# tusen-ai/simpledet

Measured on AMD Instinct MI355X. Metric: images/sec at 800x1333 FPN 512-RoI RoIAlign fwd+bwd, higher is better.
Workload: dtype f32; 1 GPU; fused FPN RoIAlign_v2 fwd+bwd, P2-P5 256ch 800x1333, N=2 img/GPU, 512 RoIs/img, 7x7x4 samples (BASELINE configs[1]); images_per_gpu=2, rois_per_image=512, argmax_state=packed u8 (decoded in backward)

## Files before the change

simpledet_amd/csrc/common.h:

```cpp
#pragma once
#include <hip/hip_runtime.h>
#include <stdint.h>
#include <stdio.h>
#include <stdarg.h>

#define SD_OK 0
#define SD_ERR_INVALID_ARG (-1)
#define SD_ERR_UNSUPPORTED (-2)
#define SD_ERR_HIP (-3)
#define SD_ERR_WORKSPACE (-4)

namespace sd {

char* err_buf();
int fail(int code, const char* fmt, ...);
void note_dispatch(const char* fmt, ...);

#define SD_REQUIRE(cond, ...)                                    \
  do {                                                           \
    if (!(cond)) return ::sd::fail(SD_ERR_INVALID_ARG, __VA_ARGS__); \
  } while (0)

#define SD_HIP_CHECK(expr)                                                              \
  do {                                                                                  \
    hipError_t e_ = (expr);                                                             \
    if (e_ != hipSuccess)                                                               \
      return ::sd::fail(SD_ERR_HIP, "%s failed: %s (%s:%d)", #expr, hipGetErrorString(e_), \
                        __FILE__, __LINE__);                                            \
  } while (0)

#define SD_LAUNCH_CHECK() SD_HIP_CHECK(hipGetLastError())

int tuning(const char* key, int dflt);
#ifdef SD_PROFILING
#define SD_PROF_TUNING(key, dflt) ::sd::tuning(key, dflt)
#define SD_ABLATE(args, bits) ((args).ablate & (bits))
#else
#define SD_PROF_TUNING(key, dflt) (dflt)
#define SD_ABLATE(args, bits) 0
// ... 134 lines not shown
```

simpledet_amd/csrc/roi_align_common.h:

```cpp
#pragma once
#include "common.h"
#include "../../include/simpledet_ops.h"
#include <float.h>
#include <math.h>
#include <type_traits>
#include <hip/hip_fp16.h>

namespace sd {

struct RoiLevels {
  const float* data[SD_MAX_FPN_LEVELS];
  int H[SD_MAX_FPN_LEVELS], W[SD_MAX_FPN_LEVELS], stride[SD_MAX_FPN_LEVELS];
  float scale[SD_MAX_FPN_LEVELS];
  int nlvl;
  float canon_scale, canon_level, k_min, k_max;
};

__device__ __forceinline__ int fpn_level(float x1, float y1, float x2, float y2,
                                         const RoiLevels& L) {
  float area = (x2 - x1 + 1.f) * (y2 - y1 + 1.f);
  float s = sqrtf(area);
  float t = floorf(L.canon_level + log2f(s / L.canon_scale + 1e-6f));
  t = t < L.k_min ? L.k_min : (t > L.k_max ? L.k_max : t);
  if (!(t == t)) return -1;
// ... 146 lines not shown

__device__ __forceinline__ void store_tap(float* dst, float v, int size) {
  int packed = -1;
  float frac = 0.f;
  if (v != -1.f) {
    const int lo = iminr(imaxr((int)floorf(v), 0), size - 1);
    const int hi = iminr(imaxr((int)ceilf(v), 0), size - 1);
    frac = (lo == hi) ? 0.5f : (v - (float)lo) / (float)(hi - lo);
    packed = lo | (hi << 16);
  }
  reinterpret_cast<int*>(dst)[0] = packed;
  dst[1] = frac;
}

constexpr int kBandThreads = 1024, kBandWaves = kBandThreads / kWave;
constexpr int kBandBufFloats = 16896;
constexpr int kBandHalo = 8;
constexpr int kBandMaxBands = 16;
constexpr int kBandNP = 4;
constexpr int kBandMaxUnits = 512;
constexpr int kBandFillCost = 140, kBandPlaneCost = 60, kBandSetupCost = 1500;
constexpr int kBandSub = 4;
constexpr int kBandFallbackWGs = 0;

typedef float v2f __attribute__((ext_vector_type(2)));

struct BandPlan {
  int owned[SD_MAX_FPN_LEVELS];
  int rows[SD_MAX_FPN_LEVELS];
  int nbands[SD_MAX_FPN_LEVELS];
  int g[SD_MAX_FPN_LEVELS];
  int unit_base[SD_MAX_FPN_LEVELS];
  int halo[SD_MAX_FPN_LEVELS];
  int nwg;
  int nunits;
  int grab;
  int gbias;
  int tail;
  int tail_planes;
  int pool;
  uint4* rowent;
  uint4* colent;
  float2* rowval;
  float2* colval;
  unsigned* items;
  int2* seg;
  unsigned char* fbflag;
  int* chan_ctr;
  int nlist, nent;
  int* ticket;
  int tail_coord, tail_lists;
};

struct BandArgs {
  FwdArgs f;
  BandPlan p;
};

struct BwdArgs {
  RoiLevels L;
  const float* dy;
  const float* ax;
  const float* ay;
  const float* rois;
  float* dx;
  int B, C, R, PP, H, W;
  float scale;
  int filter_lvl;
  int band_rows, nbands;
  int req;
  int ablate;
};

struct BwdFusedArgs {
  RoiLevels L;
  const float* dy;
  const float* ax;
  const float* ay;
  const unsigned char* amax8;
  const float* coords;
// ... 37 lines not shown
```

simpledet_amd/csrc/roi_align_fwd.hip:

```cpp
#include "roi_align_lists.h"

namespace sd {

__global__ __launch_bounds__(256) void roi_align_fwd_naive(FwdArgs a) {
  const int PP = a.PH * a.PW;
  const long count = (long)a.B * a.R * a.C * PP;
  for (long index = (long)blockIdx.x * blockDim.x + threadIdx.x; index < count;
       index += (long)gridDim.x * blockDim.x) {
    int pw = (int)(index % a.PW);
    int ph = (int)((index / a.PW) % a.PH);
    int c = (int)((index / PP) % a.C);
    int n = (int)(index / PP / a.C);
    const float* r = a.rois + (long)n * 4;
    float x1 = r[0], y1 = r[1], x2 = r[2], y2 = r[3];
    int lvl = 0;
    if (a.L.nlvl > 1) lvl = fpn_level(x1, y1, x2, y2, a.L);
    FwdOut o{0.f, -1.f, -1.f, 255};
    if (lvl >= 0) {
      int H = a.L.H[lvl], W = a.L.W[lvl];
      const float* plane = a.L.data[lvl] + ((long)(n / a.R) * a.C + c) * H * W;
      o = roi_align_fwd_elem(plane, H, W, x1, y1, x2, y2, a.L.scale[lvl], ph, pw, a.PH, a.PW);
    }
    if (a.L.nlvl > 1) o.val = o.val + 0.0f;
    a.out[index] = o.val;
// ... 413 lines not shown

template <int POOL, bool PK, bool HALF = false>
__global__ __launch_bounds__(kBandThreads) void roi_align_fwd_band(BandArgs A, BwdFusedArgs bplan) {
  using TIn = typename std::conditional<HALF, __half, float>::type;
  constexpr int AL = HALF ? 8 : 4;
  const FwdArgs& a = A.f;
  const BandPlan& P = A.p;
  constexpr int QL = POOL, IPP = kWave / QL;
  constexpr int NP = (PK && !HALF) ? kBandNP : kBandNP - 1, CAP = NP * kBandWaves * IPP;
  constexpr int PPG = POOL * POOL, PPSG = amax_stride(PPG);
  extern __shared__ __attribute__((aligned(16))) float band_smem[];
  const int tid = threadIdx.x, lane = tid & (kWave - 1);
  const int wave = __builtin_amdgcn_readfirstlane(tid / kWave);

#ifdef SD_PROFILING
  const long long t_entry = __builtin_readcyclecounter();
#endif
  __shared__ int v_unit[kBandMaxUnits], v_first[kBandMaxUnits], v_items[kBandMaxUnits];
  __shared__ int v_cost[kBandMaxUnits], v_start[kBandMaxUnits + 1];
  __shared__ int2 s_grab[2];
  __shared__ int s_pick;
  const int wg = (int)blockIdx.x - kBandFallbackWGs, nwg = (int)gridDim.x - kBandFallbackWGs;
  const int rsub = (a.R + kBandSub - 1) / kBandSub;
  auto level_of = [&](int u) {
    int l = 0;
    for (int k = 0; k < a.L.nlvl; ++k)
      if (a.L.stride[k] >= 0 && u >= P.unit_base[k]) l = k;
    return l;
  };
  __shared__ int s_nvu;
  auto wave_incl_scan = [&](int v) {
#pragma unroll
    for (int o = 1; o < kWave; o <<= 1) {
      const int t = __shfl_up(v, o);
      if (lane >= o) v += t;
    }
    return v;
  };
  static_assert(kBandMaxUnits % kWave == 0 && kBandMaxUnits / kWave <= kBandWaves, "unit table: one wave per 64 units");
  constexpr int NB = kBandMaxUnits / kWave;
  __shared__ int s_tot[NB], s_ctot[NB];
  {
    const int u = wave * kWave + lane;
    int cnt = 0, rounds = 0, lv = 0, incl = 0;
    if (wave < NB) {
      if (u < P.nunits) {
        lv = level_of(u);
#pragma unroll
        for (int j = 0; j < kBandSub; ++j) cnt += P.seg[u * kBandSub + j].y;
        rounds = (cnt + CAP - 1) / CAP;
      }
      incl = wave_incl_scan(rounds);
      if (lane == kWave - 1) s_tot[wave] = incl;
    }
    __syncthreads();
    int total = 0;
#pragma unroll
    for (int b = 0; b < NB; ++b) total += s_tot[b];
    const int n = total < kBandMaxUnits ? total : kBandMaxUnits;
    if (wave < NB) {
      int vb = incl - rounds;
#pragma unroll
      for (int b = 0; b < NB; ++b) vb += b < wave ? s_tot[b] : 0;
      for (int r = 0; r < rounds && vb + r < kBandMaxUnits; ++r) {
        const int it = cnt - r * CAP < CAP ? cnt - r * CAP : CAP;
        v_unit[vb + r] = u;
        v_first[vb + r] = r * CAP;
        v_items[vb + r] = it;
        const int cst = kBandFillCost / P.g[lv] + kBandPlaneCost + it;
        v_cost[vb + r] = P.g[lv] > 1 ? cst + cst * P.gbias / 100 : cst;
      }
    }
    __syncthreads();
    const int v = wave * kWave + lane;
    int mine = 0, cincl = 0;
    if (wave < NB) {
// ... 59 lines not shown
          best = v0 + __builtin_ctzll(__ballot(left == m));
        }
      }
      if (lane == 0) s_pick = best;
    }
    __syncthreads();
    vu = s_pick;
    if (vu < 0) break;
  }
  const int unit = v_unit[vu];
  const int lvl = level_of(unit);
  const int G = P.g[lvl], nb = P.nbands[lvl];
  const int GR = ((P.grab + G - 1) / G) * G;
  int glast = 0;
  auto next_size = [&]() { return glast >= a.C - a.C * P.tail / 100 ? (P.tail_planes < G ? P.tail_planes : G) : GR; };
  {
    const int k = grab(vu, GR);
    if (tid == 0) s_grab[0] = make_int2(k, GR);
    glast = k;
    __syncthreads();
  }
  int kcur = s_grab[0].x;
  if (kcur >= a.C) continue;
  int ck = kcur + G, cend = kcur + GR < a.C ? kcur + GR : a.C;
  int gcur = cend - kcur < G ? cend - kcur : G, gnext = 0;
  int slot = 1;
  const int ul = unit - P.unit_base[lvl];
  const int img = ul / nb, band = ul % nb;
  const int H = a.L.H[lvl], W = a.L.W[lvl], HW = H * W;
  const int r0 = band * P.owned[lvl];
  const int nrows = H - r0 < P.rows[lvl] ? H - r0 : P.rows[lvl];
  const int blen = nrows * W;
  const int bstride = HALF ? ((blen + 14) >> 3) * 8 : (blen + 4 + 3) & ~3;
  const unsigned* items = P.items + ((long)img * SD_MAX_FPN_LEVELS + lvl) * kBandSub * rsub * POOL;
  int sgs[kBandSub], sgc[kBandSub], count = 0;
#pragma unroll
  for (int j = 0; j < kBandSub; ++j) {
    const int2 sg = P.seg[unit * kBandSub + j];
    sgs[j] = j * rsub * POOL + sg.x - count;
    sgc[j] = count + sg.y;
    count += sg.y;
  }
  const int round0 = v_first[vu], nitems = v_items[vu];
#ifdef SD_PROFILING
  dbg_count += nitems;
  ++dbg_units;
  dbg_fills = 0;
  t_mark = __builtin_readcyclecounter();
  if (a.dbg && lane == 0 && wave == 0 && dbg_units <= 3) {
    long long* d = a.dbg + ((long)gridDim.x * kBandWaves + (long)blockIdx.x * 4 + (dbg_units - 1)) * 8;
    d[0] = lvl; d[2] = nitems; d[3] = t_mark; d[4] = 1;
  }
#endif
  const TIn* gbase = reinterpret_cast<const TIn*>(a.L.data[lvl]) + (long)img * a.C * HW + (long)r0 * W;
  {
    constexpr int NST = HALF ? 3 : 1;
    uint4 st[NST];
    const int n8u = (blen + 7 + 7) >> 3;
    auto fill = [&](const TIn* src, float* dst, int gcount) {
      if constexpr (!HALF) {
        int sh0 = 0;
        for (int g = 0; g < gcount; ++g) {
          const int sh = band_fill(src + (long)g * HW, blen, dst + g * bstride, wave, lane);
          if (g == 0) sh0 = sh;
        }
        return sh0;
// ... 24 lines not shown
    };
    auto fill_commit = [&](float* dst, int gcount) {
      if constexpr (HALF) {
#pragma unroll
        for (int k = 0; k < NST; ++k) {
          const int f = tid + k * kBandThreads, g = f / n8u, i = f - g * n8u;
          if (g < gcount) {
            const __half2* hp = reinterpret_cast<const __half2*>(&st[k]);
            const float2 p0 = __half22float2(hp[0]), p1 = __half22float2(hp[1]);
            const float2 p2 = __half22float2(hp[2]), p3 = __half22float2(hp[3]);
            float4* d = reinterpret_cast<float4*>(dst + g * bstride + 8 * i);
            d[0] = make_float4(p0.x, p0.y, p1.x, p1.y);
            d[1] = make_float4(p2.x, p2.y, p3.x, p3.y);
          }
        }
      }
    };
    int A0[NP], A1[NP], A2[NP], A3[NP], A4[NP], A5[NP], A6[NP], A7[NP];
    float al0[NP], al1[NP], be0[NP], be1[NP], cx0[NP], cx1[NP], cy0[NP], cy1[NP];
    int ooff[NP];
    unsigned aoff[NP];
    int flags[NP];
    bool anyd[NP];
    unsigned words[NP];
    uint4 res[NP], ces[NP];
#pragma unroll
    for (int i = 0; i < NP; ++i) {
      const int it = (wave + kBandWaves * i) * IPP + lane / QL;
      const bool valid = lane < IPP * QL && it < nitems;
      words[i] = 0;
      if (valid) {
        const int t = round0 + it;
        int o = sgs[kBandSub - 1];
#pragma unroll
        for (int j = kBandSub - 2; j >= 0; --j) o = t < sgc[j] ? sgs[j] : o;
        words[i] = items[o + t];
      }
    }
#pragma unroll
    for (int i = 0; i < NP; ++i) {
      const int it = (wave + kBandWaves * i) * IPP + lane / QL;
      const bool valid = lane < IPP * QL && it < nitems;
      const int n = words[i] & 0xffff, pp = words[i] >> 16, q = lane % QL;
      res[i] = make_uint4(0, 0, 0x7fc00000u, 0x7fc00000u);
      ces[i] = res[i];
      if (valid) {
        res[i] = P.rowent[((long)img * a.R + n) * POOL + pp];
        ces[i] = P.colent[((long)img * a.R + n) * POOL + q];
      }
    }
    int shift_next = fill(gbase + (long)kcur * HW, buf0, gcur);
    fill_commit(buf0, gcur);
    if (tid == 0) {
      const int sz = next_size();
      glast = grab(vu, sz);
      s_grab[1] = make_int2(glast, sz);
    }
#pragma unroll
    for (int i = 0; i < NP; ++i) {
      const int it = (wave + kBandWaves * i) * IPP + lane / QL;
      const bool valid = lane < IPP * QL && it < nitems;
      const unsigned word = words[i];
      const int n = word & 0xffff, pp = word >> 16, q = lane % QL;
      const uint4 re = res[i], ce = ces[i];
      if (!PK) {
        float2 rv = make_float2(0.f, 0.f), cv = rv;
        if (valid) {
          rv = P.rowval[((long)img * a.R + n) * POOL + pp];
          cv = P.colval[((long)img * a.R + n) * POOL + q];
        }
        cy0[i] = rv.x; cy1[i] = rv.y; cx0[i] = cv.x; cx1[i] = cv.y;
      }
      const int r0w = r0 * W;
      int lo0 = (int)(re.x & 0xfffff) - r0w, lo1 = (int)(re.y & 0xfffff) - r0w;
      lo0 = lo0 < 0 ? 0 : lo0;
      lo1 = lo1 < 0 ? 0 : lo1;
      const int hi0 = lo0 + ((re.x >> 20) & 1 ? W : 0), hi1 = lo1 + ((re.y >> 20) & 1 ? W : 0);
      const int left0 = ce.x & 0xfff, left1 = (ce.x >> 13) & 0xfff;
      A0[i] = (lo0 + left0) * 4; A1[i] = (lo0 + left1) * 4; A2[i] = (hi0 + left0) * 4; A3[i] = (hi0 + left1) * 4;
      A4[i] = (lo1 + left0) * 4; A5[i] = (lo1 + left1) * 4; A6[i] = (hi1 + left0) * 4; A7[i] = (hi1 + left1) * 4;
      al0[i] = __uint_as_float(re.z); al1[i] = __uint_as_float(re.w);
      be0[i] = __uint_as_float(ce.z); be1[i] = __uint_as_float(ce.w);
      const int d0 = (ce.x >> 12) & 1, d1 = (ce.x >> 25) & 1;
      const int empty = (int)(re.x >> 31) | (int)((ce.x >> 26) & 1);
      flags[i] = (valid ? 1 : 0) | d0 << 1 | d1 << 2 | empty << 3;
      anyd[i] = __ballot(valid && (d0 | d1)) != 0;
// ... 109 lines not shown
        s_grab[slot] = make_int2(grabbed, gsz);
        glast = grabbed;
      }
      kcur = knext;
      gcur = gnext;
      if (kcur >= a.C) break;
    }
#ifdef SD_PROFILING
    {
      const long long now = __builtin_readcyclecounter();
      t_comp += now - t_mark;
      t_mark = now;
    }
#endif
    __syncthreads();
  }
#ifdef SD_PROFILING
  if (a.dbg && lane == 0 && wave == 0 && dbg_units <= 3) {
    long long* d = a.dbg + ((long)gridDim.x * kBandWaves + (long)blockIdx.x * 4 + (dbg_units - 1)) * 8;
    d[1] = dbg_fills; d[5] = __builtin_readcyclecounter();
  }
#endif
  }
  {
    const int nroi = a.B * a.R;
    bool fast_void = false;
    if constexpr (!PK && !HALF) {
      fast_void = (((uintptr_t)a.out | (uintptr_t)a.ax | (uintptr_t)a.ay) & 15) == 0 && (a.C * PPG) % 4 == 0;
      if (fast_void) {
        const int n4 = a.C * PPG / 4;
        const float4 zero = make_float4(0.f, 0.f, 0.f, 0.f), neg = make_float4(-1.f, -1.f, -1.f, -1.f);
        for (int n = wg; n < nroi; n += nwg) {
          if (P.fbflag[n] != 2) continue;
          float4* o4 = reinterpret_cast<float4*>(a.out + (long)n * a.C * PPG);
          float4* x4 = reinterpret_cast<float4*>(a.ax + (long)n * a.C * PPG);
          float4* y4 = reinterpret_cast<float4*>(a.ay + (long)n * a.C * PPG);
          for (int i = tid; i < n4; i += kBandThreads) {
            o4[i] = zero;
            x4[i] = neg;
            y4[i] = neg;
          }
        }
      }
    }
    const int nsl = nwg >= a.fbslice ? a.fbslice : 1, csl = a.C / nsl, slice = wg % nsl;
    const int nslots = nwg / nsl;
    for (int n0 = wg / nsl; n0 < nroi && wg / nsl < nslots; n0 += nslots * kWave) {
      const int nl = n0 + lane * nslots;
      int myflag = nl < nroi ? P.fbflag[nl] : 0;
      if (fast_void && myflag == 2) myflag = 0;
      unsigned long long todo = __ballot(myflag != 0);
      while (todo) {
      const int src = __builtin_ctzll(todo);
      todo &= todo - 1;
      const int n = n0 + src * nslots;
      const int flag = __builtin_amdgcn_readlane(myflag, src);
      const float4 bx = *reinterpret_cast<const float4*>(a.rois + (long)n * 4);
      const int lvl = a.L.nlvl > 1 ? fpn_level(bx.x, bx.y, bx.z, bx.w, a.L) : 0;
      for (int e = tid; e < csl * PPG; e += kBandThreads) {
        const int c = slice * csl + e / PPG, g = e % PPG;
        FwdOut o{0.f, -1.f, -1.f, 255};
        if (lvl >= 0 && flag == 1) {
          const int H = a.L.H[lvl], W = a.L.W[lvl];
          o = roi_align_fwd_elem(reinterpret_cast<const TIn*>(a.L.data[lvl]) + ((long)(n / a.R) * a.C + c) * H * W,
                                 H, W, bx.x, bx.y, bx.z, bx.w, a.L.scale[lvl], g / POOL, g % POOL, POOL, POOL);
        }
        if (a.L.nlvl > 1) o.val = o.val + 0.0f;
        if constexpr (HALF) reinterpret_cast<__half*>(a.out)[((long)n * a.C + c) * PPG + g] = __float2half(o.val);
        else a.out[((long)n * a.C + c) * PPG + g] = o.val;
        if (PK) {
          a.amax8[((long)n * a.C + c) * PPSG + g] = (unsigned char)o.code;
        } else {
          a.ax[((long)n * a.C + c) * PPG + g] = o.ax;
          a.ay[((long)n * a.C + c) * PPG + g] = o.ay;
        }
      }
      }
    }
    }
  if (P.ticket) {
    const int ntasks = P.tail_coord + P.tail_lists;
    asm volatile("s_waitcnt vmcnt(0)" ::: "memory");
    static_assert(offsetof(BandArgs, f) == 0 && offsetof(FwdArgs, L) == 0, "RoiLevels leads the kernel arguments");
    const RoiLevels* geom_p = (const RoiLevels*)__builtin_amdgcn_kernarg_segment_ptr();
    asm volatile("" : "+s"(geom_p));
    const RoiLevels& geom = *geom_p;
    for (;;) {
      __syncthreads();
      if (tid == 0) s_pick = __hip_atomic_fetch_add(P.ticket, 1, __ATOMIC_RELAXED, __HIP_MEMORY_SCOPE_AGENT);
      __syncthreads();
      const int t = s_pick;
      if (t >= ntasks) break;
      if (PK && t < P.tail_coord) coords_block<POOL>(a, geom, t);
      else bwd_lists_block<POOL, POOL, kBandThreads, kMergedListSplit>(bplan, t - P.tail_coord, band_smem);
    }
  }
#ifdef SD_PROFILING
  if (a.dbg && lane == 0) {
    long long* d = a.dbg + ((long)blockIdx.x * kBandWaves + wave) * 8;
    d[0] = t_setup; d[1] = t_wait; d[2] = t_comp; d[3] = dbg_count;
    d[4] = __builtin_readcyclecounter() - t_begin; d[5] = t_begin - t_entry; d[6] = dbg_units; d[7] = t_begin;
  }
#endif
}

__global__ __launch_bounds__(512) void roi_align_fwd_quad(BandArgs A) {
  extern __shared__ __attribute__((aligned(16))) float band_smem[];
  const FwdArgs& a = A.f;
  const BandPlan& P = A.p;
  constexpr int T = 512, POOL = 7, PPG = POOL * POOL, NW = T / kWave;
  const int tid = threadIdx.x, lane = tid & (kWave - 1);
  const int wave = __builtin_amdgcn_readfirstlane(tid / kWave);
  const int G = a.C / 4;
  const int c = 4 * ((G & 7) == 0 ? (int)(blockIdx.x & 7) * (G >> 3) + (int)(blockIdx.x >> 3) : (int)blockIdx.x);
  const int img = blockIdx.y;
  const int H = a.L.H[0], W = a.L.W[0], HW = H * W;
  float4* pl = reinterpret_cast<float4*>(band_smem);
  float* st = band_smem + 4 * (HW + 1) + wave * (4 * PPG);
// ... 236 lines not shown
    P.gbias = 0;
    P.tail = 0;
    P.tail_planes = 8;
    {
      const int np = (a.amax8 && !a.half_io) ? kBandNP : kBandNP - 1;
      const long cap_launch = (long)np * kBandWaves * (kWave / POOL);
      if (units + (long)nroi * POOL / cap_launch > kBandMaxUnits) ok = false;
    }
    wg = kNumCU;
    if (ok && need <= workspace_bytes) {
      char* w = reinterpret_cast<char*>(((uintptr_t)workspace + 15) & ~(uintptr_t)15);
      P.rowent = reinterpret_cast<uint4*>(w); w += ent;
      P.colent = reinterpret_cast<uint4*>(w); w += ent;
      if (valb) {
        P.rowval = reinterpret_cast<float2*>(w); w += valb;
        P.colval = reinterpret_cast<float2*>(w); w += valb;
      }
      P.items = reinterpret_cast<unsigned*>(w); w += itemb;
      P.seg = reinterpret_cast<int2*>(w); w += segb;
      P.fbflag = reinterpret_cast<unsigned char*>(w); w += al16(nroi);
      P.chan_ctr = reinterpret_cast<int*>(w);
      P.nwg = wg;
      P.pool = POOL;
      A.f = a;
      const int nlist = a.B * a.L.nlvl * kBandSub, nent = cdiv((long)nroi * 2 * POOL, kBandThreads);
      const int ncoord = a.amax8 ? cdiv((long)nroi * 6 * POOL, kBandThreads) : 0;
      P.nlist = nlist; P.nent = nent;
      const int smem = 2 * kBandBufFloats * (int)sizeof(float);
      const bool merged = bplan && bplan->lists_units > 0 && bplan->PP == POOL * POOL;
      if (bplan_done) *bplan_done = merged;
      const int nbwd = merged ? bplan->lists_units * (kMergedListSplit + (bplan->pix_bound_words > 0 ? 1 : 0)) : 0;
      const size_t tail_lds = merged ? (size_t)(a.R + 8 + 16 + bplan->pix_bound_words) * 4 : 0;
      const bool tail = tuning("roi_align_plan_tail", 1) == 1 && ncoord + nbwd > 0 && tail_lds <= (size_t)smem;
      static const BwdFusedArgs no_plan{};
      const BwdFusedArgs& tplan = tail && merged ? *bplan : no_plan;
      if (tail) {
        P.ticket = P.chan_ctr + kBandMaxUnits;
        P.tail_coord = ncoord;
        P.tail_lists = nbwd;
      }
      if (int e = tail ? launch_fwd_prep(A, POOL, nlist + nent, nullptr, st)
                       : launch_fwd_prep(A, POOL, nlist + nent + ncoord, merged ? bplan : nullptr, st))
        return e;
      {
        const long HW0 = (long)a.L.H[0] * a.L.W[0];
        const size_t lds = (size_t)(HW0 + 1) * 16 + 8 * 4 * 49 * sizeof(float);
// ... 15 lines not shown
                                     smem));                                                      \
    hipLaunchKernelGGL(k, dim3(wg + kBandFallbackWGs), dim3(kBandThreads), smem, st, A, tplan);   \
  } while (0)
      if (a.half_io) {
#define SD_FWD_BAND_H(POOLV)                                                                      \
  do {                                                                                            \
    auto k = roi_align_fwd_band<POOLV, true, true>;                                               \
    SD_HIP_CHECK(hipFuncSetAttribute((const void*)k, hipFuncAttributeMaxDynamicSharedMemorySize,  \
                                     smem));                                                      \
    hipLaunchKernelGGL(k, dim3(wg + kBandFallbackWGs), dim3(kBandThreads), smem, st, A, tplan);   \
  } while (0)
        if (POOL == 7) SD_FWD_BAND_H(7); else SD_FWD_BAND_H(14);
#undef SD_FWD_BAND_H
      } else if (POOL == 7) {
        if (a.amax8) SD_FWD_BAND(7, true); else SD_FWD_BAND(7, false);
      } else {
        if (a.amax8) SD_FWD_BAND(14, true); else SD_FWD_BAND(14, false);
      }
#undef SD_FWD_BAND
      char tail_note[96] = "";
      if (tail) snprintf(tail_note, sizeof(tail_note), " (tail tasks: %d coordinate table + %d backward plan)", ncoord, nbwd);
      note_dispatch("sd::%s<%d> + sd::roi_align_fwd_band<%d,%s,%s>%s", merged && !tail ? "roi_prep_merged_kernel" : "roi_fwd_prep_kernel",
                    POOL, POOL, a.amax8 ? "true" : "false", a.half_io ? "true" : "false", tail_note);
      SD_LAUNCH_CHECK();
      return SD_OK;
    }
  }
  if (a.half_io)
    return fail(SD_ERR_UNSUPPORTED, "fp16 RoIAlign runs on the band-resident kernel only: it needs the workspace, "
                "7x7 or 14x14 pooling, W in [2, 4095] and roi_align_fwd = 1, roi_align_fwd_band = 1");
  note_dispatch("sd::roi_align_fwd (tiled / naive fallback kernels: no workspace or a shape the band kernel does not take)");
  if (variant >= 1 && wide && a.PH == 7 && a.PW == 7) {
    if (a.amax8)
      hipLaunchKernelGGL((roi_align_fwd_tiled<7, 7, 4, true>), dim3(cdiv(nroi, 4) * a.nslice), dim3(512), 0, st, a);
    else
      hipLaunchKernelGGL((roi_align_fwd_tiled<7, 7, 4, false>), dim3(cdiv(nroi, 4) * a.nslice), dim3(512), 0, st, a);
  } else if (variant >= 1 && wide && a.PH == 14 && a.PW == 14) {
    if (a.amax8)
      hipLaunchKernelGGL((roi_align_fwd_tiled<14, 14, 1, true>), dim3(nroi * a.nslice), dim3(512), 0,
                         st, a);
    else
      hipLaunchKernelGGL((roi_align_fwd_tiled<14, 14, 1, false>), dim3(nroi * a.nslice), dim3(512),
                         0, st, a);
  } else {
    const int grid = (int)((count + 255) / 256 < 65536 * 16 ? (count + 255) / 256 : 65536 * 16);
    hipLaunchKernelGGL(roi_align_fwd_naive, dim3(grid), dim3(256), 0, st, a);
// ... 194 lines not shown
```

simpledet_amd/csrc/roi_align_prep.hip:

```cpp
#include "roi_align_lists.h"

namespace sd {

template <int POOL>
__device__ __forceinline__ void band_prep_block(const BandArgs& A, const int pblock, int nlist, int nent) {
  const FwdArgs& a = A.f;
  const BandPlan& P = A.p;
  const int tid = threadIdx.x, lane = tid & (kWave - 1);
  constexpr int LPR = POOL <= 8 ? 8 : 16;
  constexpr int RPP = kBandThreads / LPR;
  if (pblock < nlist) {
    __shared__ int hist[kBandMaxBands], cursor[kBandMaxBands];
    const int sub = pblock % kBandSub, lvl = (pblock / kBandSub) % a.L.nlvl;
    const int img = pblock / (kBandSub * a.L.nlvl);
    if (a.L.stride[lvl] < 0) return;
    int first_valid = 0;
    while (a.L.stride[first_valid] < 0) ++first_valid;
    const int H = a.L.H[lvl], W = a.L.W[lvl], nb = P.nbands[lvl], owned = P.owned[lvl];
    const float scale = a.L.scale[lvl];
    const int rsub = (a.R + kBandSub - 1) / kBandSub;
    const int rbeg = sub * rsub, rend = rbeg + rsub < a.R ? rbeg + rsub : a.R;
    if (tid < kBandMaxBands) hist[tid] = 0;
    __syncthreads();
    const int rr = tid / LPR, p = tid % LPR;
    unsigned* items = P.items + (((long)img * SD_MAX_FPN_LEVELS + lvl) * kBandSub + sub) * rsub * POOL;
    auto classify = [&](int n) -> int {
      int band = -1;
      bool bad = false, mine = false, emp_r = true, emp_c = true;
      int lv = -2;
      if (n < rend) {
        const float4 bx = *reinterpret_cast<const float4*>(a.rois + ((long)img * a.R + n) * 4);
        lv = a.L.nlvl > 1 ? fpn_level(bx.x, bx.y, bx.z, bx.w, a.L) : 0;
        mine = lv == lvl;
        if (mine && p < POOL) {
          float val[2], frac[2];
          int offr[4], offc[4];
          const int cr = axis_samples(p, POOL, bx.y, bx.w, scale, H, 1, val, frac, offr);
          const int cc = axis_samples(p, POOL, bx.x, bx.z, scale, W, 1, val, frac, offc);
          bad = cr >= 3 || cc >= 3;
          emp_r = cr < 0;
          emp_c = cc < 0;
          band = 0;
          if (cr >= 1) {
            const int first = offr[0], last = cr >= 2 ? offr[3] : offr[1];
            if (nb > 1 && last - first > P.halo[lvl]) bad = true;
            band = first / owned;
          }
        }
      }
      const unsigned long long bm = __ballot(bad);
      const int sh = (lane / LPR) * LPR;
      const unsigned long long rmask = (1ull << LPR) - 1;
      bool roi_bad = ((bm >> sh) & rmask) != 0;
      const bool all_r = ((__ballot(!emp_r) >> sh) & rmask) == 0, all_c = ((__ballot(!emp_c) >> sh) & rmask) == 0;
      const bool roi_void = mine && (all_r || all_c);
      roi_bad = roi_bad || roi_void;
      if (n < rend && p == 0) {
        if (mine) P.fbflag[(long)img * a.R + n] = roi_void ? 2 : (roi_bad ? 1 : 0);
        else if (lv < 0 && lvl == first_valid) P.fbflag[(long)img * a.R + n] = 2;
      }
      return roi_bad ? -2 : band;
    };
    constexpr int KP = 4;
    int keep[KP];
    const int npass = (rend - rbeg + RPP - 1) / RPP;
#pragma unroll
    for (int k = 0; k < KP; ++k) {
      keep[k] = -1;
      if (k < npass) {
        keep[k] = classify(rbeg + k * RPP + rr);
        if (keep[k] >= 0) atomicAdd(&hist[keep[k]], 1);
      }
    }
    for (int k = KP; k < npass; ++k) {
      const int band = classify(rbeg + k * RPP + rr);
      if (band >= 0) atomicAdd(&hist[band], 1);
    }
    __syncthreads();
    if (tid == 0) {
      int run = 0;
      for (int b = 0; b < nb; ++b) {
        cursor[b] = run;
        P.seg[(P.unit_base[lvl] + img * nb + b) * kBandSub + sub] = make_int2(run, hist[b]);
        run += hist[b];
      }
    }
    __syncthreads();
    auto emit = [&](int n, int band) {
      unsigned long long todo = __ballot(band >= 0);
      while (todo) {
        const int src = __builtin_ctzll(todo);
        const int bb = __builtin_amdgcn_readlane(band, src);
        const unsigned long long m = __ballot(band == bb);
        int base = 0;
        if (lane == src) base = atomicAdd(&cursor[bb], __popcll(m));
        base = __builtin_amdgcn_readlane(base, src);
        if (band == bb)
          items[base + __builtin_amdgcn_mbcnt_hi((unsigned)(m >> 32), __builtin_amdgcn_mbcnt_lo((unsigned)m, 0))] =
              (unsigned)n | ((unsigned)p << 16);
        todo &= ~m;
      }
    };
#pragma unroll
    for (int k = 0; k < KP; ++k)
      if (k < npass) emit(rbeg + k * RPP + rr, keep[k]);
    for (int k = KP; k < npass; ++k) {
      const int n = rbeg + k * RPP + rr;
      emit(n, classify(n));
    }
    return;
  }
  if (pblock == nlist && tid < kBandMaxUnits) P.chan_ctr[tid] = 0;
  if (pblock == nlist && tid == 0 && P.ticket) *P.ticket = 0;
  const int eb = pblock - nlist;
  const int nroi = a.B * a.R;
  if (eb < nent) {
    const long e = (long)eb * kBandThreads + tid;
    if (e >= (long)nroi * 2 * POOL) return;
    const int p = (int)(e % POOL), ax = (int)((e / POOL) % 2), n = (int)(e / (2 * POOL));
    const float4 bx = *reinterpret_cast<const float4*>(a.rois + (long)n * 4);
    const int lvl = a.L.nlvl > 1 ? fpn_level(bx.x, bx.y, bx.z, bx.w, a.L) : 0;
    if (lvl < 0) return;
    const int H = a.L.H[lvl], W = a.L.W[lvl];
    float val[2] = {0.f, 0.f}, frac[2] = {0.f, 0.f};
    int off[4];
    const int cnt = ax == 0 ? axis_samples(p, POOL, bx.y, bx.w, a.L.scale[lvl], H, W, val, frac, off)
                            : axis_samples(p, POOL, bx.x, bx.z, a.L.scale[lvl], W, 1, val, frac, off);
    const float qnan = __int_as_float(0x7fc00000);
    const bool v0 = cnt >= 1, v1 = cnt >= 2;
    uint4 en;
    if (ax == 0) {
// ... 61 lines not shown
```

simpledet_amd/csrc/runtime.hip:

```cpp
#include "common.h"
#include <stdarg.h>
#include "../../include/simpledet_ops.h"
#include <atomic>
#include <string.h>
#include <hip/hip_fp16.h>

namespace sd {

char* err_buf() {
  static thread_local char buf[512] = {0};
  return buf;
}

int fail(int code, const char* fmt, ...) {
  va_list ap;
  va_start(ap, fmt);
  vsnprintf(err_buf(), 512, fmt, ap);
  va_end(ap);
  return code;
}

namespace {
struct Knob {
  const char* key;
  std::atomic<int> value;
  std::atomic<bool> set;
  Knob(const char* k, int v, bool s) : key(k), value(v), set(s) {}
};
Knob g_knobs[] = {
    {"roi_align_fwd", 0, false},
    {"roi_align_fwd_band", 0, false},
    {"roi_align_fwd_quad", 0, false},
    {"roi_align_plan_tail", 0, false},
    {"roi_align_bwd", 0, false},
    {"roi_align_bwd_flt4", 0, false},
    {"roi_align_bwd_fx", 0, false},
    {"roi_align_bwd_pixbound", 0, false},
    {"roi_align_bwd_lists", 0, false},
    {"roi_pool_fwd", 0, false},
    {"roi_pool_bwd", 0, false},
    {"deform_psroi_bwd_patch", 0, false},
    {"proposal_topk", 0, false},
    {"soft_nms_threads", 0, false},
    {"deform_gemm_split", 0, false},
    {"deform_gemm_vecstore", 0, false},
    {"deform_gemm_nt", 0, false},
    {"deform_gemm_ksplit", 0, false},
    {"dcn_im2col", 0, false},
    {"dcn_window", 0, false},
    {"dcn_im2col_pipe", 0, false},
    {"dcn_col2im", 0, false},
    {"dcn_col2im_fx", 0, false},
    {"dcn_coord", 0, false},
    {"dcn_fused", 0, false},
    {"dcn_fused_tile", 0, false},
// ... 83 lines not shown
  SD_REQUIRE(src && dst, "null buffer");
  SD_REQUIRE(((uintptr_t)src & 15) == 0 && ((uintptr_t)dst & 15) == 0, "buffers must be 16-byte aligned");
  sd::cast_h2f_kernel<<<sd::kNumCU * 8, 256, 0, (hipStream_t)stream>>>((const __half*)src, dst, n);
  SD_LAUNCH_CHECK();
  return SD_OK;
}

extern "C" int sd_cast_f32_to_f16(const float* src, void* dst, size_t n, int req, void* stream) {
  if (n == 0 || req == SD_REQ_NULL) return SD_OK;
  SD_REQUIRE(src && dst, "null buffer");
  SD_REQUIRE(req == SD_REQ_WRITE || req == SD_REQ_ADD, "req must be write or add");
  sd::cast_f2h_kernel<<<sd::kNumCU * 8, 256, 0, (hipStream_t)stream>>>(src, (__half*)dst, n, req == SD_REQ_ADD);
  SD_LAUNCH_CHECK();
  return SD_OK;
}

extern "C" int sd_stream_synchronize(void* stream) {
  SD_HIP_CHECK(hipStreamSynchronize((hipStream_t)stream));
  return SD_OK;
}

namespace sd {
static thread_local char g_dispatch[256] = {0};
void note_dispatch(const char* fmt, ...) {
  va_list ap;
  va_start(ap, fmt);
  vsnprintf(g_dispatch, sizeof(g_dispatch), fmt, ap);
  va_end(ap);
}
}

extern "C" const char* sd_last_error(void) { return sd::err_buf(); }
extern "C" const char* sd_last_dispatch(void) { return sd::g_dispatch; }
extern "C" int sd_abi_version(void) { return SD_ABI_VERSION; }

extern "C" int sd_set_tuning(const char* key, int value) {
  if (!key) return sd::fail(SD_ERR_INVALID_ARG, "null tuning key");
  for (auto& k : sd::g_knobs)
    if (!strcmp(k.key, key)) {
      k.value.store(value, std::memory_order_relaxed);
      k.set.store(true, std::memory_order_release);
      return SD_OK;
    }
  return sd::fail(SD_ERR_INVALID_ARG, "unknown tuning key '%s'", key);
}

extern "C" int sd_get_tuning(const char* key, int* value) {
  if (!key || !value) return sd::fail(SD_ERR_INVALID_ARG, "null argument");
  for (auto& k : sd::g_knobs)
    if (!strcmp(k.key, key)) {
      *value = k.set.load() ? k.value.load() : -1;
      return SD_OK;
    }
  return sd::fail(SD_ERR_INVALID_ARG, "unknown tuning key '%s'", key);
}
```

Measured before the change: 11000 images/s.

## Schedule flagged RoI fallback work through the dynamic task counter

```diff
diff --git a/simpledet_amd/csrc/common.h b/simpledet_amd/csrc/common.h
--- a/simpledet_amd/csrc/common.h
+++ b/simpledet_amd/csrc/common.h
@@ -15,6 +15,8 @@
 char* err_buf();
 int fail(int code, const char* fmt, ...);
 void note_dispatch(const char* fmt, ...);
+int* dispatch_flag_words(hipStream_t st);
+void note_dispatch_flagged(int slices, bool tasks);
 
 #define SD_REQUIRE(cond, ...)                                    \
   do {                                                           \
diff --git a/simpledet_amd/csrc/roi_align_common.h b/simpledet_amd/csrc/roi_align_common.h
--- a/simpledet_amd/csrc/roi_align_common.h
+++ b/simpledet_amd/csrc/roi_align_common.h
@@ -192,6 +192,7 @@
 constexpr int kBandFillCost = 140, kBandPlaneCost = 60, kBandSetupCost = 1500;
 constexpr int kBandSub = 4;
 constexpr int kBandFallbackWGs = 0;
+constexpr int kBandFlagWords = 512;
 
 typedef float v2f __attribute__((ext_vector_type(2)));
 
@@ -215,6 +216,7 @@
   float2* colval;
   unsigned* items;
   int2* seg;
+  int* flagged_host;
   unsigned char* fbflag;
   int* chan_ctr;
   int nlist, nent;
@@ -226,6 +228,19 @@
   FwdArgs f;
   BandPlan p;
 };
+
+__device__ __forceinline__ int2 band_seg_first(int items, int n1, int n2) {
+  return make_int2((int)(0x80000000u | (unsigned)n1 | (unsigned)n2 << 15), items);
+}
+__device__ __forceinline__ int2 band_seg(const BandPlan& P, int unit, int j, int* n1 = nullptr, int* n2 = nullptr) {
+  int2 sg = P.seg[unit * kBandSub + j];
+  if (sg.x < 0) {
+    if (n1) *n1 += sg.x & 0x7fff;
+    if (n2) *n2 += (sg.x >> 15) & 0x7fff;
+    sg.x = 0;
+  }
+  return sg;
+}
 
 struct BwdArgs {
   RoiLevels L;
diff --git a/simpledet_amd/csrc/roi_align_fwd.hip b/simpledet_amd/csrc/roi_align_fwd.hip
--- a/simpledet_amd/csrc/roi_align_fwd.hip
+++ b/simpledet_amd/csrc/roi_align_fwd.hip
@@ -459,10 +459,14 @@
   __shared__ int s_pick;
   const int wg = (int)blockIdx.x - kBandFallbackWGs, nwg = (int)gridDim.x - kBandFallbackWGs;
   const int rsub = (a.R + kBandSub - 1) / kBandSub;
+  auto unit_geom = [&](int u, int& l, int& base, int& nbv) {
+    l = 0; base = 0; nbv = 1;
+    for (int k = 0; k < a.L.nlvl; ++k)
+      if (a.L.stride[k] >= 0 && u >= P.unit_base[k]) { l = k; base = P.unit_base[k]; nbv = P.nbands[k]; }
+  };
   auto level_of = [&](int u) {
-    int l = 0;
-    for (int k = 0; k < a.L.nlvl; ++k)
-      if (a.L.stride[k] >= 0 && u >= P.unit_base[k]) l = k;
+    int l, base, nbv;
+    unit_geom(u, l, base, nbv);
     return l;
   };
   __shared__ int s_nvu;
@@ -477,18 +481,28 @@
   static_assert(kBandMaxUnits % kWave == 0 && kBandMaxUnits / kWave <= kBandWaves, "unit table: one wave per 64 units");
   constexpr int NB = kBandMaxUnits / kWave;
   __shared__ int s_tot[NB], s_ctot[NB];
+  __shared__ int s_ftot[2][NB];
   {
     const int u = wave * kWave + lane;
     int cnt = 0, rounds = 0, lv = 0, incl = 0;
     if (wave < NB) {
+      int f1 = 0, f2 = 0;
       if (u < P.nunits) {
         lv = level_of(u);
 #pragma unroll
-        for (int j = 0; j < kBandSub; ++j) cnt += P.seg[u * kBandSub + j].y;
+        for (int j = 0; j < kBandSub; ++j) {
+          cnt += band_seg(P, u, j, &f1, &f2).y;
+        }
         rounds = (cnt + CAP - 1) / CAP;
       }
       incl = wave_incl_scan(rounds);
-      if (lane == kWave - 1) s_tot[wave] = incl;
+      f1 = wave_sum_i32(f1);
+      f2 = wave_sum_i32(f2);
+      if (lane == kWave - 1) {
+        s_tot[wave] = incl;
+        s_ftot[0][wave] = f1;
+        s_ftot[1][wave] = f2;
+      }
     }
     __syncthreads();
     int total = 0;
@@ -594,9 +608,6 @@
   }
   int kcur = s_grab[0].x;
   if (kcur >= a.C) continue;
-  int ck = kcur + G, cend = kcur + GR < a.C ? kcur + GR : a.C;
-  int gcur = cend - kcur < G ? cend - kcur : G, gnext = 0;
-  int slot = 1;
   const int ul = unit - P.unit_base[lvl];
   const int img = ul / nb, band = ul % nb;
   const int H = a.L.H[lvl], W = a.L.W[lvl], HW = H * W;
@@ -608,12 +619,31 @@
   int sgs[kBandSub], sgc[kBandSub], count = 0;
 #pragma unroll
   for (int j = 0; j < kBandSub; ++j) {
-    const int2 sg = P.seg[unit * kBandSub + j];
+    const int2 sg = band_seg(P, unit, j);
     sgs[j] = j * rsub * POOL + sg.x - count;
     sgc[j] = count + sg.y;
     count += sg.y;
   }
   const int round0 = v_first[vu], nitems = v_items[vu];
+  unsigned words[NP];
+  int vlane = lane;
+  asm volatile("" : "+v"(vlane));
+#pragma unroll
+  for (int i = 0; i < NP; ++i) {
+    const int it = (wave + kBandWaves * i) * IPP + vlane / QL;
+    const bool valid = vlane < IPP * QL && it < nitems;
+    words[i] = 0;
+    if (valid) {
+      const int t = round0 + it;
+      int o = sgs[kBandSub - 1];
+#pragma unroll
+      for (int j = kBandSub - 2; j >= 0; --j) o = t < sgc[j] ? sgs[j] : o;
+      words[i] = items[o + t];
+    }
+  }
+  int ck = kcur + G, cend = kcur + GR < a.C ? kcur + GR : a.C;
+  int gcur = cend - kcur < G ? cend - kcur : G, gnext = 0;
+  int slot = 1;
 #ifdef SD_PROFILING
   dbg_count += nitems;
   ++dbg_units;
@@ -684,26 +714,12 @@
     unsigned aoff[NP];
     int flags[NP];
     bool anyd[NP];
-    unsigned words[NP];
     uint4 res[NP], ces[NP];
 #pragma unroll
     for (int i = 0; i < NP; ++i) {
-      const int it = (wave + kBandWaves * i) * IPP + lane / QL;
-      const bool valid = lane < IPP * QL && it < nitems;
-      words[i] = 0;
-      if (valid) {
-        const int t = round0 + it;
-        int o = sgs[kBandSub - 1];
-#pragma unroll
-        for (int j = kBandSub - 2; j >= 0; --j) o = t < sgc[j] ? sgs[j] : o;
-        words[i] = items[o + t];
-      }
-    }
-#pragma unroll
-    for (int i = 0; i < NP; ++i) {
-      const int it = (wave + kBandWaves * i) * IPP + lane / QL;
-      const bool valid = lane < IPP * QL && it < nitems;
-      const int n = words[i] & 0xffff, pp = words[i] >> 16, q = lane % QL;
+      const int it = (wave + kBandWaves * i) * IPP + vlane / QL;
+      const bool valid = vlane < IPP * QL && it < nitems;
+      const int n = words[i] & 0xffff, pp = words[i] >> 16, q = vlane % QL;
       res[i] = make_uint4(0, 0, 0x7fc00000u, 0x7fc00000u);
       ces[i] = res[i];
       if (valid) {
@@ -720,10 +736,10 @@
     }
 #pragma unroll
     for (int i = 0; i < NP; ++i) {
-      const int it = (wave + kBandWaves * i) * IPP + lane / QL;
-      const bool valid = lane < IPP * QL && it < nitems;
+      const int it = (wave + kBandWaves * i) * IPP + vlane / QL;
+      const bool valid = vlane < IPP * QL && it < nitems;
       const unsigned word = words[i];
-      const int n = word & 0xffff, pp = word >> 16, q = lane % QL;
+      const int n = word & 0xffff, pp = word >> 16, q = vlane % QL;
       const uint4 re = res[i], ce = ces[i];
       if (!PK) {
         float2 rv = make_float2(0.f, 0.f), cv = rv;
@@ -879,7 +895,36 @@
   }
 #endif
   }
-  {
+  const int nsl = nwg >= a.fbslice ? a.fbslice : 1, csl = a.C / nsl;
+  auto flagged_slice = [&](int n, int flag, int slice) {
+    float4 bx = make_float4(0.f, 0.f, 0.f, 0.f);
+    int lvl = -1;
+    if (flag == 1) {
+      bx = *reinterpret_cast<const float4*>(a.rois + (long)n * 4);
+      lvl = a.L.nlvl > 1 ? fpn_level(bx.x, bx.y, bx.z, bx.w, a.L) : 0;
+    }
+    for (int e = tid; e < csl * PPG; e += kBandThreads) {
+      const int c = slice * csl + e / PPG, g = e % PPG;
+      FwdOut o{0.f, -1.f, -1.f, 255};
+      if (lvl >= 0) {
+        const int H = a.L.H[lvl], W = a.L.W[lvl];
+        o = roi_align_fwd_elem(reinterpret_cast<const TIn*>(a.L.data[lvl]) + ((long)(n / a.R) * a.C + c) * H * W,
+                               H, W, bx.x, bx.y, bx.z, bx.w, a.L.scale[lvl], g / POOL, g % POOL, POOL, POOL);
+      }
+      if (a.L.nlvl > 1) o.val = o.val + 0.0f;
+      if constexpr (HALF) reinterpret_cast<__half*>(a.out)[((long)n * a.C + c) * PPG + g] = __float2half(o.val);
+      else a.out[((long)n * a.C + c) * PPG + g] = o.val;
+      if (PK) {
+        a.amax8[((long)n * a.C + c) * PPSG + g] = (unsigned char)o.code;
+      } else {
+        a.ax[((long)n * a.C + c) * PPG + g] = o.ax;
+        a.ay[((long)n * a.C + c) * PPG + g] = o.ay;
+      }
+    }
+  };
+  bool tasks = false;
+  if constexpr (PK) tasks = P.ticket != nullptr;
+  if (!tasks) {
     const int nroi = a.B * a.R;
     bool fast_void = false;
     if constexpr (!PK && !HALF) {
@@ -900,8 +945,7 @@
         }
       }
     }
-    const int nsl = nwg >= a.fbslice ? a.fbslice : 1, csl = a.C / nsl, slice = wg % nsl;
-    const int nslots = nwg / nsl;
+    const int slice = wg % nsl, nslots = nwg / nsl;
     for (int n0 = wg / nsl; n0 < nroi && wg / nsl < nslots; n0 += nslots * kWave) {
       const int nl = n0 + lane * nslots;
       int myflag = nl < nroi ? P.fbflag[nl] : 0;
@@ -911,32 +955,85 @@
       const int src = __builtin_ctzll(todo);
       todo &= todo - 1;
       const int n = n0 + src * nslots;
-      const int flag = __builtin_amdgcn_readlane(myflag, src);
-      const float4 bx = *reinterpret_cast<const float4*>(a.rois + (long)n * 4);
-      const int lvl = a.L.nlvl > 1 ? fpn_level(bx.x, bx.y, bx.z, bx.w, a.L) : 0;
-      for (int e = tid; e < csl * PPG; e += kBandThreads) {
-        const int c = slice * csl + e / PPG, g = e % PPG;
-        FwdOut o{0.f, -1.f, -1.f, 255};
-        if (lvl >= 0 && flag == 1) {
-          const int H = a.L.H[lvl], W = a.L.W[lvl];
-          o = roi_align_fwd_elem(reinterpret_cast<const TIn*>(a.L.data[lvl]) + ((long)(n / a.R) * a.C + c) * H * W,
-                                 H, W, bx.x, bx.y, bx.z, bx.w, a.L.scale[lvl], g / POOL, g % POOL, POOL, POOL);
-        }
-        if (a.L.nlvl > 1) o.val = o.val + 0.0f;
-        if constexpr (HALF) reinterpret_cast<__half*>(a.out)[((long)n * a.C + c) * PPG + g] = __float2half(o.val);
-        else a.out[((long)n * a.C + c) * PPG + g] = o.val;
-        if (PK) {
-          a.amax8[((long)n * a.C + c) * PPSG + g] = (unsigned char)o.code;
-        } else {
-          a.ax[((long)n * a.C + c) * PPG + g] = o.ax;
-          a.ay[((long)n * a.C + c) * PPG + g] = o.ay;
-        }
-      }
-      }
-    }
-    }
+      flagged_slice(n, __builtin_amdgcn_readlane(myflag, src), slice);
+      }
+    }
+  }
   if (P.ticket) {
-    const int ntasks = P.tail_coord + P.tail_lists;
+    int nex = 0, nvo = 0;
+    if (tasks) {
+#pragma unroll
+      for (int b = 0; b < NB; ++b) {
+        nex += s_ftot[0][b];
+        nvo += s_ftot[1][b];
+      }
+      nex = __builtin_amdgcn_readfirstlane(nex);
+      nvo = __builtin_amdgcn_readfirstlane(nvo);
+    }
+    const int t_ex = P.tail_lists, t_co = t_ex + nex * nsl, t_vo = t_co + P.tail_coord, ntasks = t_vo + nvo;
+    constexpr int NSLOT = kBandMaxUnits * kBandSub;
+    static_assert(NSLOT == 2 * kBandThreads, "flagged prefix: two slots per thread");
+    int* tab_e = reinterpret_cast<int*>(band_smem);
+    int* tab_v = tab_e + NSLOT + 1;
+    int* tab_w = tab_v + NSLOT + 1;
+    bool have_table = false;
+    auto build_table = [&]() {
+      int e2[2], v2[2];
+#pragma unroll
+      for (int k = 0; k < 2; ++k) {
+        const int s = 2 * tid + k;
+        e2[k] = v2[k] = 0;
+        if (s < P.nunits * kBandSub) band_seg(P, s / kBandSub, s % kBandSub, &e2[k], &v2[k]);
+      }
+      const int es = e2[0] + e2[1], vs = v2[0] + v2[1];
+      const int ei = wave_incl_scan(es), vi = wave_incl_scan(vs);
+      if (lane == kWave - 1) {
+        tab_w[wave] = ei;
+        tab_w[kBandWaves + wave] = vi;
+      }
+      __syncthreads();
+      int eo = ei - es, vo = vi - vs;
+      for (int b = 0; b < wave; ++b) {
+        eo += tab_w[b];
+        vo += tab_w[kBandWaves + b];
+      }
+      tab_e[2 * tid] = eo;
+      tab_e[2 * tid + 1] = eo + e2[0];
+      tab_v[2 * tid] = vo;
+      tab_v[2 * tid + 1] = vo + v2[0];
+      if (tid == kBandThreads - 1) {
+        tab_e[NSLOT] = eo + es;
+        tab_v[NSLOT] = vo + vs;
+      }
+      __syncthreads();
+    };
+    auto flagged_task = [&](int t) {
+      const bool exact = t < t_co;
+      const int rr = exact ? (t - t_ex) / nsl : t - t_vo, slice = exact ? t - t_ex - rr * nsl : 0;
+      const int* tb = exact ? tab_e : tab_v;
+      int lo = 0, hi = NSLOT;
+      while (hi - lo > 1) {
+        const int mid = (lo + hi) >> 1;
+        if (tb[mid] <= rr) lo = mid; else hi = mid;
+      }
+      const int pos = rr - tb[lo] + (exact ? 0 : tab_e[lo + 1] - tab_e[lo]);
+      const int u = lo / kBandSub, j = lo % kBandSub;
+      int l, base, nbv;
+      unit_geom(u, l, base, nbv);
+      const int img = (u - base) / nbv;
+      const unsigned word = P.items[(((long)img * SD_MAX_FPN_LEVELS + l) * kBandSub + j + 1) * rsub * POOL - 1 - pos];
+      const int n = img * a.R + (int)(word & 0xffff);
+      if (exact) {
+        flagged_slice(n, 1, slice);
+      } else {
+        for (int e = tid; e < a.C * PPG; e += kBandThreads) {
+          const int c = e / PPG, g = e % PPG;
+          if constexpr (HALF) reinterpret_cast<__half*>(a.out)[(long)n * a.C * PPG + e] = __float2half(0.f);
+          else a.out[(long)n * a.C * PPG + e] = 0.f;
+          a.amax8[((long)n * a.C + c) * PPSG + g] = (unsigned char)255;
+        }
+      }
+    };
     asm volatile("s_waitcnt vmcnt(0)" ::: "memory");
     static_assert(offsetof(BandArgs, f) == 0 && offsetof(FwdArgs, L) == 0, "RoiLevels leads the kernel arguments");
     const RoiLevels* geom_p = (const RoiLevels*)__builtin_amdgcn_kernarg_segment_ptr();
@@ -946,11 +1043,27 @@
       __syncthreads();
       if (tid == 0) s_pick = __hip_atomic_fetch_add(P.ticket, 1, __ATOMIC_RELAXED, __HIP_MEMORY_SCOPE_AGENT);
       __syncthreads();
-      const int t = s_pick;
+      const int t = __builtin_amdgcn_readfirstlane(s_pick);
       if (t >= ntasks) break;
-      if (PK && t < P.tail_coord) coords_block<POOL>(a, geom, t);
-      else bwd_lists_block<POOL, POOL, kBandThreads, kMergedListSplit>(bplan, t - P.tail_coord, band_smem);
-    }
+      if (t < t_ex) {
+        bwd_lists_block<POOL, POOL, kBandThreads, kMergedListSplit>(bplan, t, band_smem);
+      } else if (PK && t >= t_co && t < t_vo) {
+        coords_block<POOL>(a, geom, t - t_co);
+      } else if (PK) {
+        if (!have_table) build_table();
+        have_table = true;
+        flagged_task(t);
+      }
+    }
+  }
+  if (P.flagged_host && blockIdx.x == 0 && tid == 0) {
+    int f1 = 0, f2 = 0;
+    for (int b = 0; b < NB; ++b) {
+      f1 += s_ftot[0][b];
+      f2 += s_ftot[1][b];
+    }
+    P.flagged_host[0] = f1;
+    P.flagged_host[1] = f2;
   }
 #ifdef SD_PROFILING
   if (a.dbg && lane == 0) {
@@ -1233,6 +1346,7 @@
       P.chan_ctr = reinterpret_cast<int*>(w);
       P.nwg = wg;
       P.pool = POOL;
+      P.flagged_host = tuning("roi_align_flag_report", 1) == 1 ? dispatch_flag_words(st) : nullptr;
       A.f = a;
       const int nlist = a.B * a.L.nlvl * kBandSub, nent = cdiv((long)nroi * 2 * POOL, kBandThreads);
       const int ncoord = a.amax8 ? cdiv((long)nroi * 6 * POOL, kBandThreads) : 0;
@@ -1294,6 +1408,7 @@
       if (tail) snprintf(tail_note, sizeof(tail_note), " (tail tasks: %d coordinate table + %d backward plan)", ncoord, nbwd);
       note_dispatch("sd::%s<%d> + sd::roi_align_fwd_band<%d,%s,%s>%s", merged && !tail ? "roi_prep_merged_kernel" : "roi_fwd_prep_kernel",
                     POOL, POOL, a.amax8 ? "true" : "false", a.half_io ? "true" : "false", tail_note);
+      if (P.flagged_host) note_dispatch_flagged(wg >= a.fbslice ? a.fbslice : 1, tail && a.amax8);
       SD_LAUNCH_CHECK();
       return SD_OK;
     }
diff --git a/simpledet_amd/csrc/roi_align_prep.hip b/simpledet_amd/csrc/roi_align_prep.hip
--- a/simpledet_amd/csrc/roi_align_prep.hip
+++ b/simpledet_amd/csrc/roi_align_prep.hip
@@ -6,11 +6,13 @@
 __device__ __forceinline__ void band_prep_block(const BandArgs& A, const int pblock, int nlist, int nent) {
   const FwdArgs& a = A.f;
   const BandPlan& P = A.p;
-  const int tid = threadIdx.x, lane = tid & (kWave - 1);
+  const int tid = threadIdx.x, lane = tid & (kWave - 1), wave = tid / kWave;
   constexpr int LPR = POOL <= 8 ? 8 : 16;
   constexpr int RPP = kBandThreads / LPR;
   if (pblock < nlist) {
     __shared__ int hist[kBandMaxBands], cursor[kBandMaxBands];
+    __shared__ unsigned fmask[2 * kBandFlagWords];
+    __shared__ int fcount[2];
     const int sub = pblock % kBandSub, lvl = (pblock / kBandSub) % a.L.nlvl;
     const int img = pblock / (kBandSub * a.L.nlvl);
     if (a.L.stride[lvl] < 0) return;
@@ -21,13 +23,15 @@
     const int rsub = (a.R + kBandSub - 1) / kBandSub;
     const int rbeg = sub * rsub, rend = rbeg + rsub < a.R ? rbeg + rsub : a.R;
     if (tid < kBandMaxBands) hist[tid] = 0;
+    const int fw = (rsub + 31) >> 5;
+    for (int i = tid; i < 2 * fw; i += kBandThreads) fmask[i] = 0;
     __syncthreads();
     const int rr = tid / LPR, p = tid % LPR;
     unsigned* items = P.items + (((long)img * SD_MAX_FPN_LEVELS + lvl) * kBandSub + sub) * rsub * POOL;
     auto classify = [&](int n) -> int {
       int band = -1;
       bool bad = false, mine = false, emp_r = true, emp_c = true;
-      int lv = -2;
+      int lv = -2, myfl = 0;
       if (n < rend) {
         const float4 bx = *reinterpret_cast<const float4*>(a.rois + ((long)img * a.R + n) * 4);
         lv = a.L.nlvl > 1 ? fpn_level(bx.x, bx.y, bx.z, bx.w, a.L) : 0;
@@ -56,8 +60,23 @@
       const bool roi_void = mine && (all_r || all_c);
       roi_bad = roi_bad || roi_void;
       if (n < rend && p == 0) {
-        if (mine) P.fbflag[(long)img * a.R + n] = roi_void ? 2 : (roi_bad ? 1 : 0);
-        else if (lv < 0 && lvl == first_valid) P.fbflag[(long)img * a.R + n] = 2;
+        int fl = -1;
+        if (mine) fl = roi_void ? 2 : (roi_bad ? 1 : 0);
+        else if (lv < 0 && lvl == first_valid) fl = 2;
+        if (fl >= 0) P.fbflag[(long)img * a.R + n] = (unsigned char)fl;
+        myfl = fl > 0 ? fl : 0;
+      }
+      const unsigned long long f1 = __ballot(myfl == 1), f2 = __ballot(myfl == 2);
+      if (lane == 0 && (f1 | f2)) {
+        unsigned m1 = 0, m2 = 0;
+#pragma unroll
+        for (int i = 0; i < kWave / LPR; ++i) {
+          m1 |= (unsigned)((f1 >> (i * LPR)) & 1) << i;
+          m2 |= (unsigned)((f2 >> (i * LPR)) & 1) << i;
+        }
+        const int w = (n - rbeg) >> 5, sh5 = (n - rbeg) & 31;
+        if (m1) atomicOr(&fmask[w], m1 << sh5);
+        if (m2) atomicOr(&fmask[fw + w], m2 << sh5);
       }
       return roi_bad ? -2 : band;
     };
@@ -77,15 +96,30 @@
       if (band >= 0) atomicAdd(&hist[band], 1);
     }
     __syncthreads();
+    int2* seg0 = P.seg + (P.unit_base[lvl] + img * nb) * kBandSub + sub;
     if (tid == 0) {
       int run = 0;
       for (int b = 0; b < nb; ++b) {
         cursor[b] = run;
-        P.seg[(P.unit_base[lvl] + img * nb + b) * kBandSub + sub] = make_int2(run, hist[b]);
+        if (b > 0) seg0[b * kBandSub] = make_int2(run, hist[b]);
         run += hist[b];
       }
     }
+    if (wave == 1) {
+      int c1 = 0, c2 = 0;
+      for (int j = lane; j < fw; j += kWave) {
+        c1 += __popc(fmask[j]);
+        c2 += __popc(fmask[fw + j]);
+      }
+      c1 = wave_sum_i32(c1);
+      c2 = wave_sum_i32(c2);
+      if (lane == 0) {
+        fcount[0] = c1;
+        fcount[1] = c2;
+      }
+    }
     __syncthreads();
+    if (tid == 0) seg0[0] = band_seg_first(hist[0], fcount[0], fcount[1]);
     auto emit = [&](int n, int band) {
       unsigned long long todo = __ballot(band >= 0);
       while (todo) {
@@ -107,6 +141,20 @@
     for (int k = KP; k < npass; ++k) {
       const int n = rbeg + k * RPP + rr;
       emit(n, classify(n));
+    }
+    for (int i = tid; i < 2 * fw && P.ticket; i += kBandThreads) {
+      unsigned m = fmask[i];
+      if (m == 0) continue;
+      int pos = 0;
+      for (int j = 0; j < i; ++j) pos += __popc(fmask[j]);
+      const unsigned tag = i < fw ? 1u << 16 : 2u << 16;
+      const int nbase = rbeg + ((i < fw ? i : i - fw) << 5);
+      while (m) {
+        const int bit = __builtin_ctz(m);
+        m &= m - 1;
+        items[rsub * POOL - 1 - pos] = (unsigned)(nbase + bit) | tag;
+        ++pos;
+      }
     }
     return;
   }
diff --git a/simpledet_amd/csrc/runtime.hip b/simpledet_amd/csrc/runtime.hip
--- a/simpledet_amd/csrc/runtime.hip
+++ b/simpledet_amd/csrc/runtime.hip
@@ -2,6 +2,7 @@
 #include <stdarg.h>
 #include "../../include/simpledet_ops.h"
 #include <atomic>
+#include <mutex>
 #include <string.h>
 #include <hip/hip_fp16.h>
 
@@ -31,6 +32,7 @@
     {"roi_align_fwd", 0, false},
     {"roi_align_fwd_band", 0, false},
     {"roi_align_fwd_quad", 0, false},
+    {"roi_align_flag_report", 0, false},
     {"roi_align_plan_tail", 0, false},
     {"roi_align_bwd", 0, false},
     {"roi_align_bwd_flt4", 0, false},
@@ -160,16 +162,55 @@
 
 namespace sd {
 static thread_local char g_dispatch[256] = {0};
+static thread_local int* g_flag_words = nullptr;
+static thread_local int g_flag_slices = 0;
+static thread_local bool g_flag_tasks = false;
+static thread_local char g_dispatch_full[384] = {0};
 void note_dispatch(const char* fmt, ...) {
   va_list ap;
   va_start(ap, fmt);
   vsnprintf(g_dispatch, sizeof(g_dispatch), fmt, ap);
   va_end(ap);
+  g_flag_slices = 0;
+}
+constexpr int kFlagSlots = 64;
+static std::mutex g_flag_mu;
+static int* g_flag_pool = nullptr;
+static int g_flag_used = 0;
+int* dispatch_flag_words(hipStream_t st) {
+  if (!g_flag_words) {
+    std::lock_guard<std::mutex> lock(g_flag_mu);
+    if (!g_flag_pool) {
+      hipStreamCaptureStatus cs = hipStreamCaptureStatusNone;
+      void* p = nullptr;
+      if (hipStreamIsCapturing(st, &cs) != hipSuccess || cs != hipStreamCaptureStatusNone ||
+          hipHostMalloc(&p, kFlagSlots * 2 * sizeof(int), hipHostMallocDefault) != hipSuccess) {
+        (void)hipGetLastError();
+        return nullptr;
+      }
+      g_flag_pool = reinterpret_cast<int*>(p);
+    }
+    if (g_flag_used >= kFlagSlots) return nullptr;
+    g_flag_words = g_flag_pool + 2 * g_flag_used++;
+    g_flag_words[0] = g_flag_words[1] = -1;
+  }
+  return g_flag_words;
+}
+void note_dispatch_flagged(int slices, bool tasks) {
+  g_flag_slices = g_flag_words ? slices : 0;
+  g_flag_tasks = tasks;
 }
 }
 
 extern "C" const char* sd_last_error(void) { return sd::err_buf(); }
-extern "C" const char* sd_last_dispatch(void) { return sd::g_dispatch; }
+extern "C" const char* sd_last_dispatch(void) {
+  if (!sd::g_flag_slices) return sd::g_dispatch;
+  const volatile int* w = sd::g_flag_words;
+  snprintf(sd::g_dispatch_full, sizeof(sd::g_dispatch_full), "%s [flagged RoIs: %d exact path + %d constant, x %d channel slices, %s]",
+           sd::g_dispatch, w[0], w[1], sd::g_flag_slices,
+           sd::g_flag_tasks ? "drawn from the task counter" : "walked in fixed shares");
+  return sd::g_dispatch_full;
+}
 extern "C" int sd_abi_version(void) { return SD_ABI_VERSION; }
 
 extern "C" int sd_set_tuning(const char* key, int value) {
```

Measured after the change: 11220 images/s (median of 4 runs). +2.0%, better.
